# spacejam/tla-rust

Measured on AMD Instinct MI355X. Metric: distinct states/sec, raft.tla (3 servers), higher is better.
Workload: dtype u64

## Files before the change

### __graft_entry__.py

```python
import subprocess
import sys
from pathlib import Path

ROOT = Path(__file__).resolve().parent
sys.path.insert(0, str(ROOT))
sys.path.insert(0, str(ROOT / "tests"))


def build() -> None:
    import tla_rust_amd.build as b
    so = b.build()
    assert so.exists()
    subprocess.run(["make", "-s", "-C", str(ROOT / "oracle")], check=True)
    import helpers
    helpers.build_shim()
    helpers.build_fakerccl()
    helpers.build_tlaeval_door()
    import sgraph
    sgraph.build()
    import sfgraph
    sfgraph.build()
    import ufgraph
    ufgraph.build()
    import sideshim
    sideshim.build()
    sideshim.build_host()
    import behshim
    behshim.build()
    behshim.build_devices()
    import tla_rust_amd
    tla_rust_amd.lib()


def smoke() -> None:
    import helpers
    import tla_rust_amd as amd
    assert amd.device_count() >= 1, "smoke() needs a HIP device"
    for spec, params in (("atomic_add", [10]), ("pcal_intro", [0, 1, 20, 2]), ("raft", [2, 2, 2, 9, 1, 1]), ("ssi", [2, 2, 127, 0])):
        eng = amd.Engine(spec, params, device=0, table_capacity=1 << 20, arena_capacity=1 << 18, chunk_states=1 << 14)
        r = eng.run()
        o = helpers.oracle_run(spec, params)
        assert (r.distinct, r.generated, r.depth, r.verdict, r.levels) == \
               (o["distinct"], o["generated"], o["depth"], o["verdict"], o["levels"]), (spec, dict(r), o)
        eng.close()
        print(f"smoke {spec}{params}: {r.distinct} distinct / {r.generated} generated / depth {r.depth} == oracle")
    params = [0, 3, 2, 3, 15, 3, 1]
    eng = amd.Engine("paxos", params, device=0, table_capacity=1 << 20, arena_capacity=1 << 18, deadlock=False)
    r = eng.run()
    o = helpers.oracle_run("paxos", params, check_deadlock=False)
    assert (r.distinct, r.generated, r.depth, r.verdict, r.levels) == (o["distinct"], o["generated"], o["depth"], o["verdict"], o["levels"])
    assert r.distinct == 17153
    eng.close()
    print(f"smoke paxos{params}: {r.distinct} orbits / {r.generated} generated / depth {r.depth} == oracle == reference text")
    sys.path.insert(0, str(ROOT / "oracle"))
    from tla_eval import Checker
    text = (ROOT / "specs" / "pluscal" / "cas_counter.tla").read_text()
    prog = amd.Program(text, (ROOT / "specs" / "pluscal" / "cas_counter.cfg").read_text())
    eng = amd.Engine("pcal", prog.params, device=0, table_capacity=1 << 20, arena_capacity=1 << 18, chunk_states=1 << 12)
    r = eng.run()
    o = Checker(prog.translated(), constants={"Workers": 2, "N": 2}).run_levels(invariants=["NeverTooMany", "SeenIsOld"])
    assert (r.distinct, r.generated, r.depth, r.verdict, r.levels) == (o["distinct"], o["generated"], o["depth"], o["verdict"], o["levels"])
    eng.close()
# ... 9 lines not shown
```

### include/tlamc.h

```cpp
#ifndef TLAMC_H
#define TLAMC_H
#include <stddef.h>
#include <stdint.h>

#ifdef __cplusplus
extern "C" {
#endif

#define MC_OK 0
#define MC_EBADCFG (-1)
#define MC_EHIP (-2)
#define MC_EOVERFLOW (-3)
#define MC_ETABLEFULL (-4)
#define MC_EARENA (-5)
#define MC_ERCCL (-6)
#define MC_ESTATE (-7)
#define MC_EPARSE (-8)
#define MC_ENOSPEC (-9)
#define MC_EROUTE (-10)

#define MC_V_OK 0
#define MC_V_INVARIANT 1
#define MC_V_ASSERT 2
#define MC_V_DEADLOCK 3
#define MC_V_SPECERR 4
#define MC_V_BUDGET 5
#define MC_V_ASSUME 6
#define MC_V_LIVENESS 7

#define MC_SPEC_ATOMIC_ADD 1
#define MC_SPEC_PCAL_INTRO 2
#define MC_SPEC_RAFT 3

#define MC_SPEC_SSI 4

#define MC_SPEC_PCAL 5

#define MC_SPEC_PAXOS 6

typedef struct {
    uint32_t spec_id;
    uint32_t nparams;
    int64_t params[16];
} mc_spec_desc;

#define MC_F_DEADLOCK 1u
#define MC_F_TRACE 2u
#define MC_F_TIMING 4u
#define MC_F_MATRIX 8u
#define MC_F_NOPROBE 16u
#define MC_F_NOFAMILY 32u
#define MC_F_OCC3 2048u
#define MC_F_NOINWAVE 65536u
#define MC_F_WAVETAIL 131072u
#define MC_F_PARK 32768u
#define MC_F_NOFILTER 8192u
#define MC_F_SYNCPROBE 4096u
#define MC_F_PROGRESS 16384u
#define MC_F_NOBATCH 256u
#define MC_F_UNVERIFIED 512u
#define MC_F_JIT 262144u
#define MC_F_GENERIC 128u
#define MC_F_STRONGFAIR 33554432u
#define MC_F_LABELFAIR 134217728u
#define MC_F_COVERAGE 16777216u
#define MC_F_CONTINUE 67108864u

typedef struct {
    int32_t device;
    uint32_t flags;
    uint64_t table_capacity;
    uint64_t arena_capacity;
    uint64_t chunk_states;
    uint64_t max_levels;
    uint64_t max_distinct;
    uint32_t shard_rank;
    uint32_t shard_count;
} mc_config;

#define MC_MAX_LEVELS 4096

typedef struct {
    uint64_t distinct;
    uint64_t generated;
    uint64_t queue_left;
    uint32_t depth;
    int32_t verdict;
    int32_t violated_invariant;
    uint32_t trace_len;
    uint32_t levels;
// ... 371 lines not shown
```

### tla_rust_amd/build.py

```python
import os
import subprocess
from pathlib import Path

PKG = Path(__file__).resolve().parent
CSRC = PKG / "csrc"
OUT = PKG / "_build"
LIB = OUT / "libtlamc.so"
CLI = OUT / "mc"

SOURCES = ["engine.hip", "frontend.cpp"]

ENGINE_BASE = ["engine.hip", "hip_owned.h", "engine_kernels.h", "engine_sim.h", "sim_walk.h", "engine_behaviours.h", "behaviour.h", "engine_coverage.h", "coverage.h", "engine_violations.h", "violations.h",
               "engine_graph.h",
               "graph.h", "liveness.h", "live_query.h", "state_graph.h", "spec_gen.h", "mc_common.h", "spec_registry.h", "../../include/tlamc.h"]
ENGINE_OWN = {0: ["spec_pluscal.h", "spec_raft.h", "spec_raft_packed.h", "spec_ssi.h", "spec_vm.h", "spec_vm_cfg.h", "spec_paxos.h", "engine_pairs.h"], 7: ["spec_paxos.h"], 1: ["spec_pluscal.h"],
              2: ["spec_raft.h"], 3: ["spec_raft.h"], 4: ["spec_raft.h"], 5: ["spec_ssi.h", "engine_pairs.h"], 6: ["spec_vm.h", "spec_vm_cfg.h"],
              12: ["spec_raft.h", "spec_raft_packed.h"], 13: ["spec_raft.h", "spec_raft_packed.h"]}
STATE_GRAPH_DEPS = ["state_graph.hip", "state_graph.h", "engine_live.h", "hip_owned.h", "liveness.h", "live_query.h", "graph.h", "coverage.h", "mc_common.h", "spec_registry.h",
                    "spec_gen.h", "spec_pluscal.h", "spec_raft.h", "spec_raft_packed.h", "spec_ssi.h", "spec_vm.h", "spec_vm_cfg.h", "spec_paxos.h", "../../include/tlamc.h"]


def _stale(target, deps):
    if not target.exists():
        return True
    t = target.stat().st_mtime
    return any(d.stat().st_mtime > t for d in deps)


def build(force=False, verbose=False):
    OUT.mkdir(exist_ok=True)
    hipcc = os.environ.get("HIPCC", "/opt/rocm/bin/hipcc")
    deps = list(CSRC.glob("*")) + [PKG.parent / "include" / "tlamc.h"]
    srcs = [str(CSRC / s) for s in SOURCES if (CSRC / s).exists()]
    common = [hipcc, "--offload-arch=gfx950", "-O3", "-std=c++17", "-fPIC", "-Wno-unused-value", "-Wno-unused-result",
              "-I", str(PKG.parent / "include")]
    if os.environ.get("TLAMC_LINE_TABLES"):
        common.append("-gline-tables-only")
    if os.environ.get("TLAMC_EXTRA_DEFS"):
        common += os.environ["TLAMC_EXTRA_DEFS"].split()
    if os.environ.get("TLAMC_PHASE_PROF"):
        common.append("-DMC_PHASE_PROF")
    jobs, objs = [], []
    for tu in sorted(ENGINE_OWN):
        obj = OUT / f"engine_tu{tu}.o"
        objs.append(obj)
# ... 48 lines not shown
```

### tla_rust_amd/csrc/engine.hip

```cpp
#include <hip/hip_runtime.h>

#include <algorithm>
#include <chrono>
#include <memory>
#include <type_traits>
#include <string>
#include <vector>

#include "spec_registry.h"
#include "hip_owned.h"

namespace mc {

#ifndef MC_TU
#define MC_TU -1
#endif
}
#include "engine_kernels.h"
#include "engine_pairs.h"
#include "engine_sim.h"
#include "engine_behaviours.h"
#include "engine_coverage.h"
#include "engine_violations.h"
#include "engine_graph.h"
#include "state_graph.h"
namespace mc {

struct EngineBase {
    DevBuf<int32_t> owned_device_blob;
    uint64_t program_hash = 0;
    mc_progress_fn progress_fn = nullptr;
    void *progress_user = nullptr;
    double progress_interval = 1.0;
    std::chrono::steady_clock::time_point progress_last;
    bool stop_requested = false;
    void report_progress(uint32_t levels, uint64_t generated, uint64_t distinct, uint64_t queue) {
        if (!progress_fn) return;
        const auto now = std::chrono::steady_clock::now();
        if (std::chrono::duration<double>(now - progress_last).count() < progress_interval) return;
        progress_last = now;
        progress_fn(progress_user, levels, generated, distinct, queue);
    }
    virtual ~EngineBase() = default;
    virtual int run(mc_result *out) = 0;
    virtual int step(uint32_t levels, mc_result *out) = 0;
    virtual int trace(uint8_t *states_out, int32_t *actions_out, size_t *n_inout) = 0;
    virtual int kernel_stats(mc_kernel_stats *out) = 0;
    virtual int read_states(uint64_t first, uint64_t count, uint8_t *out) = 0;
    virtual int debug_reexpand(unsigned extra_flags, double *ms) = 0;
    virtual int debug_phases(uint64_t *out48, int reset) = 0;
    virtual int debug_flags(uint32_t set, uint32_t clear) = 0;
// ... 710 lines not shown
        const unsigned gm = bx < 8 * 256 ? (bx + 7) / 8 : 256;
        return gm ? gm : 1u;
    }
    void finish_materialise(uint64_t chunk_base, uint64_t ncols, unsigned parity, hipStream_t expanded_on = nullptr) {
        if (pairs_only()) return;
        unsigned gm = mat_grid(ncols);
        if (fr.mat_inwave_level) {
            const uint64_t want = (fr.mat_list_hint * 4 + 255) / 256;
            const unsigned per_seg = (unsigned)((want + NSHARD - 1) / NSHARD);
            if (per_seg < gm) gm = per_seg ? per_seg : 1u;
        }
        hipEventRecord(ev_e[parity].get(), expanded_on ? expanded_on : stream.s);
        hipStreamWaitEvent(stream2, ev_e[parity].get(), 0);
        timed(2, 0, [&] {
            hipLaunchKernelGGL(k_materialise<S>, dim3(gm, NSHARD), dim3(256), 0, stream2, prm, d_arena, chunk_base, d_newlist,
                               seg_cap, arena_cap, d_parent, d_pslot, d_ctr, parity, (const LevelCtl *)nullptr, (const uint64_t *)d_newfp);
        }, stream2);
        hipLaunchKernelGGL(k_commit, dim3(1), dim3(1), 0, stream2, d_ctr, parity);
        hipEventRecord(ev_m[parity].get(), stream2);
        static const bool serial = getenv("TLAMC_SERIAL") != nullptr;
        if (serial) hipStreamSynchronize(stream2);
    }
    void enqueue_blind_level(uint64_t max_states) {
        const uint64_t ncols = max_states + 64;
        RouteArgs rt{};
        rt.lc = d_lc;
        rt.new_fp = d_newfp;
        set_inwave(rt);
        const unsigned sg = slices_for(ncols, true);
        const bool dl = sg > 1 && (cfg.flags & MC_F_DEADLOCK);
        if (dl) { rt.succ = d_nsl; hipMemsetAsync(d_nsl, 0, ncols * sizeof(uint16_t), stream); }
        const unsigned lflags = cfg.flags | ((cfg.flags & MC_F_PARK) ? MC_FI_PARK : 0u);
        timed(0, 0, [&] {
            launch_expand<S, false>(!(cfg.flags & MC_F_NOFAMILY), lflags, ncols, stream, sg, prm, (const uint64_t *)d_arena,
                                    (uint64_t)0, (uint64_t)0, ncols, d_table.p, seen_arg(), d_newlist.p, seg_cap, d_ctr.p, cfg.flags, rt, 0u);
            if (dl) hipLaunchKernelGGL(k_deadlock_slices, dim3((unsigned)((ncols + 255) / 256)), dim3(256), 0, stream, (const uint16_t *)d_nsl,
                                       (uint64_t)0, (uint64_t)0, ncols, (const LevelCtl *)d_lc, d_ctr);
        });
        if (!pairs_only()) timed(2, 0, [&] {
            hipLaunchKernelGGL(k_materialise<S>, dim3(32, NSHARD), dim3(256), 0, stream, prm, d_arena, (uint64_t)0, d_newlist, seg_cap,
                               arena_cap, d_parent, d_pslot, d_ctr, 0u, (const LevelCtl *)d_lc, (const uint64_t *)d_newfp);
        });
        hipLaunchKernelGGL(k_end_level, dim3(1), dim3(1), 0, stream, d_ctr, d_lc);
    }

    template <bool INIT>
    void finish_chunk(uint64_t chunk_base_or_first, uint64_t ncols, unsigned rows) {
        const unsigned bx = (unsigned)((ncols + 255) / 256);
        timed(1, ncols * rows, [&] {
            hipLaunchKernelGGL(k_insert, dim3(bx, rows), dim3(256), 0, stream, d_cand, row_stride, ncols, d_nsl, d_table,
                               seen_arg(), d_newlist, d_ctr);
        });
        const unsigned gm = bx < 2048 ? bx : 2048;
        timed(2, 0, [&] {
            if (INIT)
                hipLaunchKernelGGL(k_init_materialise<S>, dim3(gm), dim3(256), 0, stream, prm, d_arena, chunk_base_or_first,
                                   d_inittmp, d_newlist, arena_cap, d_parent, d_pslot, d_ctr);
            else
                hipLaunchKernelGGL(k_materialise<S>, dim3(gm, 1), dim3(256), 0, stream, prm, d_arena, chunk_base_or_first,
                                   d_newlist, seg_cap, arena_cap, d_parent, d_pslot, d_ctr, 0u, (const LevelCtl *)nullptr, (const uint64_t *)nullptr);
        });
        hipLaunchKernelGGL(k_commit, dim3(1), dim3(1), 0, stream, d_ctr, 0u);
    }

    int seed_init(unsigned rank, unsigned count, bool resuming, bool in_place, std::chrono::steady_clock::time_point *t0) {
        if (!in_place) HIP_TRY(hipMemsetAsync(d_table, 0, table_cap * sizeof(uint64_t), stream));
        HIP_TRY(hipMemsetAsync(d_ctr, 0, sizeof(DevCounters), stream));
// ... 126 lines not shown
                alloc_atomic = lvl_inwave;
            }
            prev_frontier = hi - lo;
            fr.mat_inwave_level = lvl_inwave;
            unsigned chunk_no = 0;
            const bool two_streams = stream_b && !use_matrix && hi - lo > chunk && !(slices_for(chunk, false) > 1 && (cfg.flags & MC_F_DEADLOCK));
            if (two_streams) {
                hipEventRecord(ev_level.get(), stream);
                hipStreamWaitEvent(stream_b, ev_level.get(), 0);
            }
            for (uint64_t c0 = lo; c0 < hi; ++chunk_no) {
                const unsigned parity = chunk_no & 1u;
                const uint64_t base = c0 & ~63ull;
                uint64_t c1 = base + chunk;
                if (c1 > hi) c1 = hi;
                const uint64_t ncols = ((c1 - base) + 63) & ~63ull;
                if (use_matrix) {
                    timed(0, c1 - c0, [&] {
                        hipLaunchKernelGGL(k_expand<S>, dim3((unsigned)((ncols + 255) / 256)), dim3(256), 0, stream, prm, d_arena,
                                           c0, c1, d_cand, row_stride, ncols, d_nsl, d_ctr, cfg.flags);
                    });
                    finish_chunk<false>(base, ncols, max_slots);
                } else {
                    hipStream_t es = two_streams && parity ? stream_b.s : stream.s;
                    if (chunk_no >= 2) hipStreamWaitEvent(es, ev_m[parity].get(), 0);
                    RouteArgs rt_new{};
                    rt_new.new_fp = d_newfp;
                    if (lvl_inwave) set_inwave(rt_new);
                    const unsigned sg = slices_for(ncols, false);
                    const bool dl = sg > 1 && (cfg.flags & MC_F_DEADLOCK);
                    if (dl) { rt_new.succ = d_nsl; hipMemsetAsync(d_nsl, 0, ncols * sizeof(uint16_t), es); }
                    const unsigned lflags = cfg.flags | (lvl_inwave && park_levels ? MC_FI_PARK : 0u);
                    timed(0, c1 - c0, [&] {
                        launch_expand<S, false>(!(cfg.flags & MC_F_NOFAMILY), lflags, ncols, es, sg, prm,
                                                (const uint64_t *)d_arena, c0, c1, ncols, d_table.p, seen_arg(), d_newlist.p, seg_cap, d_ctr.p,
                                                cfg.flags, rt_new, parity);
                        if (dl) hipLaunchKernelGGL(k_deadlock_slices, dim3((unsigned)((ncols + 255) / 256)), dim3(256), 0, es,
                                                   (const uint16_t *)d_nsl, c0, c1, ncols, (const LevelCtl *)nullptr, d_ctr);
                    }, es);
                    finish_materialise(base, ncols, parity, es);
                }
                c0 = c1;
            }
            if ((rc = read_counters())) return rc;
            if ((rc = check_dev_error())) return rc;
            {
                const uint64_t via = h_ctr->via_list - via_seen;
                via_seen = h_ctr->via_list;
                const double growth = hi > lo ? (double)(h_ctr->arena_next - hi) / (double)(hi - lo) : 1.0;
                fr.mat_list_hint = (uint64_t)((double)(via / (chunk_no ? chunk_no : 1u)) * (growth > 1.0 ? growth : 1.0)) + 1;
            }
            if (cov.on) { cov_generated(lo, hi); cov_distinct(hi, h_ctr->arena_next); }
            if (vio.on && h_ctr->viol_key != ~0ull && (rc = viol_level(lo, hi, h_ctr->arena_next, true))) return rc;
            if ((rc = close_level(lo, hi, h_ctr->arena_next, level, out))) return rc;
            progress(level, lo, hi);
        }
        if (cov.on && (rc = cov_end())) return rc;
        if (hi > lo && h_ctr->viol_key == ~0ull && !fr.stop_frontier && (rc = check_frontier(lo, hi))) return rc;
        if (vio.on && hi > lo && !vio.fatal && h_ctr->viol_key != ~0ull && (rc = viol_level(lo, hi, hi, false))) return rc;
        const unsigned long long run_key = vio.on && vio.have_first ? vio.first_key : h_ctr->viol_key;
        const auto t1 = std::chrono::steady_clock::now();
        out->seconds = std::chrono::duration<double>(t1 - t0).count();
        out->distinct = h_ctr->arena_next;
        fr.last_distinct = h_ctr->arena_next;
        kstat[2].units = h_ctr->arena_next;
        out->generated = 0;
        fr.cells = 0;
// ... 296 lines not shown
                e1 = hipMemcpyAsync(out + off * W * sizeof(uint64_t), tmp, n * W * sizeof(uint64_t), hipMemcpyDeviceToHost, stream);
                e2 = hipStreamSynchronize(stream);
            }
            if (e1 != hipSuccess || e2 != hipSuccess) { set_error("read_states: copy failed"); return MC_EHIP; }
        }
        return MC_OK;
    }
    int debug_flags(uint32_t set, uint32_t clear) override { cfg.flags = (cfg.flags & ~clear) | set; return MC_OK; }
    int seen_layout(uint64_t *buckets, uint32_t *slots) override {
        *buckets = seen_arg() & ~SEEN_SPARSE;
        *slots = seen_sparse ? MC_SPARSE_SLOTS : 8;
        return MC_OK;
    }
    int debug_phases(uint64_t *out48, int reset) override {
#ifdef MC_PHASE_PROF
        HIP_TRY(hipSetDevice(cfg.device));
        HIP_TRY(hipDeviceSynchronize());
        HIP_TRY(hipMemcpyFromSymbol(out48, HIP_SYMBOL(g_phase), 48 * sizeof(uint64_t)));
        if (reset) { static const unsigned long long zero[48] = {}; HIP_TRY(hipMemcpyToSymbol(HIP_SYMBOL(g_phase), zero, sizeof zero)); }
        return MC_OK;
#else
        (void)out48; (void)reset;
        set_error("the library was built without MC_PHASE_PROF");
        return MC_ESTATE;
#endif
    }
    int debug_reexpand(unsigned extra_flags, double *ms) override {
        HIP_TRY(hipSetDevice(cfg.device));
        Event a(hipEventDefault), b(hipEventDefault);
        HIP_TRY(hipEventRecord(a.get(), stream));
        for (uint64_t c0 = 0; c0 < fr.last_distinct; c0 += chunk) {
            const uint64_t c1 = c0 + chunk < fr.last_distinct ? c0 + chunk : fr.last_distinct;
            const uint64_t ncols = ((c1 - c0) + 63) & ~63ull;
            launch_expand<S, false>(!((cfg.flags | extra_flags) & MC_F_NOFAMILY), cfg.flags | extra_flags, ncols, stream, 0u, prm,
                                    (const uint64_t *)d_arena, c0, c1, ncols, d_table.p, seen_arg(), d_newlist.p, seg_cap, d_ctr.p,
                                    cfg.flags | extra_flags, RouteArgs{}, 0u);
            hipLaunchKernelGGL(k_commit, dim3(1), dim3(1), 0, stream, d_ctr, 0u);
        }
        HIP_TRY(hipEventRecord(b.get(), stream));
        HIP_TRY(hipStreamSynchronize(stream));
        float t = 0;
        HIP_TRY(hipEventElapsedTime(&t, a.get(), b.get()));
        *ms = t;
        return MC_OK;
    }
    int shard_alloc(ShSlot &q, uint64_t send_cap) {
        const unsigned P = nranks();
        if (send_cap > q.pend_src.n) {
            q.rt_fp.reset(); q.rt_src.reset(); q.pend_src.reset();
            q.rt_subcap = (send_cap / (P * NSHARD)) * 2 + 4096;
            HIP_TRY(q.rt_fp.alloc((size_t)P * NSHARD * q.rt_subcap));
            HIP_TRY(q.rt_src.alloc((size_t)P * NSHARD * q.rt_subcap));
            HIP_TRY(q.pend_src.alloc(send_cap));
        }
        HIP_TRY(q.rt_cur.reserve((size_t)(P * NSHARD)));
        if (send_cap > sh.d_incl.n) {
            sh.d_new_src.reset(); sh.d_incl.reset();
            HIP_TRY(sh.d_new_src.alloc(send_cap));
            HIP_TRY(sh.d_incl.alloc(send_cap));
        }
        HIP_TRY(sh.d_ends.reserve(8));
        HIP_TRY(sh.h_ends.reserve(8));
        HIP_TRY(sh.h_cur.reserve((size_t)8 * NSHARD));
        return MC_OK;
    }
    static int refuse_packed() {
        if constexpr (PackedRows<S>::value) { set_error("this engine of generated code stores rows packed to its program's cell ranges and serves ONE GPU: create a sharded engine with shard_count > 1 (or $TLAMC_JIT_PACK=0)"); return MC_EBADCFG; }
// ... 106 lines not shown
            hipLaunchKernelGGL(k_materialise<S>, dim3(mat_grid(q.ncols), NSHARD), dim3(256), 0, stream2, prm, d_arena, q.chunk_base, d_newlist, seg_cap,
                               arena_cap, d_parent, d_pslot, d_ctr, slot, (const LevelCtl *)nullptr, (const uint64_t *)d_newfp);
        }, stream2);
        hipLaunchKernelGGL(k_commit, dim3(1), dim3(1), 0, stream2, d_ctr, slot);
        append_end(stream2);
        HIP_TRY(hipEventRecord(sh.ev_mat[slot].get(), stream2));
        return MC_OK;
    }
    int shard_expand_launch(unsigned slot, uint64_t first, uint64_t count, uint64_t send_cap) override {
        HIP_TRY(hipSetDevice(cfg.device));
        if (slot > 1) { set_error("shard_expand: slot must be 0 or 1"); return MC_EBADCFG; }
        ShSlot &q = sh.sl[slot];
        const unsigned P = nranks();
        int rc = shard_alloc(q, send_cap);
        if (rc) return rc;
        q.pend_total = 0;
        q.count = count;
        q.launched = true;
        for (unsigned t = 0; t <= 8; t++) q.pend_off.off[t] = 0;
        if (first + count > sh.hi - sh.lo) { set_error("shard_expand: chunk outside the local frontier"); return MC_EBADCFG; }
        if (count > chunk) { set_error("shard_expand: chunk larger than chunk_states"); return MC_EBADCFG; }
        if (!count) return MC_OK;
        if (sh.ev_slot[slot].made()) HIP_TRY(hipStreamWaitEvent(stream, sh.ev_slot[slot].get(), 0));
        if (sh.ev_mat[slot].made()) HIP_TRY(hipStreamWaitEvent(stream, sh.ev_mat[slot].get(), 0));
        HIP_TRY(hipMemsetAsync(q.rt_cur, 0, (size_t)(P * NSHARD) * sizeof(PaddedCounter), stream));
        const uint64_t c0 = sh.lo + first, c1 = c0 + count, base = c0 & ~63ull;
        const uint64_t ncols = ((c1 - base) + 63) & ~63ull;
        q.chunk_base = base;
        RouteArgs rt{P, q.rt_cur, q.rt_fp, q.rt_src, q.rt_subcap};
        rt.my_rank = cfg.shard_rank;
        rt.new_fp = d_newfp;
        q.ncols = ncols;
        timed(0, count, [&] {
            launch_expand<S, true>(!(cfg.flags & MC_F_NOFAMILY), cfg.flags, ncols, stream, 0u, prm,
                                   (const uint64_t *)d_arena, c0, c1, ncols, d_table.p, seen_arg(), d_newlist.p, seg_cap, d_ctr.p, cfg.flags, rt, slot);
        });
        return MC_OK;
    }
    int shard_expand_finish(unsigned slot, uint64_t *send_fp, uint64_t send_cap, uint64_t *send_counts) override {
        HIP_TRY(hipSetDevice(cfg.device));
        if (slot > 1 || !sh.sl[slot].launched) { set_error("shard_expand_finish: no expand in flight for this slot"); return MC_EBADCFG; }
        ShSlot &q = sh.sl[slot];
        q.launched = false;
        const unsigned P = nranks();
        for (unsigned t = 0; t < P; t++) send_counts[t] = 0;
        if (!q.count) return MC_OK;
        PaddedCounter *cur = sh.h_cur;
        HIP_TRY(hipMemcpyAsync(cur, q.rt_cur, (size_t)(P * NSHARD) * sizeof(PaddedCounter), hipMemcpyDeviceToHost, stream));
        HIP_TRY(hipMemcpyAsync(h_ctr, d_ctr, sizeof(DevCounters), hipMemcpyDeviceToHost, stream));
        HIP_TRY(hipStreamSynchronize(stream));
        int rc;
        if ((rc = check_dev_error())) return rc;
        uint64_t total = 0;
        for (unsigned t = 0; t < P; t++) {
            q.pend_off.off[t] = total;
            for (unsigned x = 0; x < NSHARD; x++) {
                if (cur[t * NSHARD + x].v > q.rt_subcap) { set_error("shard_expand: route bucket overflow (raise send_cap)"); return MC_EROUTE; }
                send_counts[t] += cur[t * NSHARD + x].v;
            }
            total += send_counts[t];
        }
        for (unsigned t = P; t <= 8; t++) q.pend_off.off[t] = total;
        if (total >= (1ull << 31)) { set_error("shard_expand: more than 2^31 candidates in one round (lower chunk_states)"); return MC_EARENA; }
        if (total > q.pend_src.n) { set_error("shard_expand: more candidates in one round than the slot's pending list holds (raise the fan-out allowance)"); return MC_EROUTE; }
        if (total > send_cap) { set_error("shard_expand: send buffer too small (raise the fan-out allowance)"); return MC_EROUTE; }
        q.pend_total = total;
        if (q.keep_pending) {
// ... 1025 lines not shown
```

Baseline: 4.234 billion.

## Add specialized production expand kernel for small Raft specs with cold kernarg reloads

Adds a dedicated family-expand kernel for Raft specs with at most three servers, used when no generic or debug flags are set. Rarely used arguments are re-read from the kernarg segment only where needed, to cut register pressure and spills. The kernel also uses a batched seen-set insert: one vectorized first-round bucket probe per lane, with a non-inlined narrow fallback that only runs when the first round cannot place the fingerprint. This duplicates a large kernel body, which raises maintenance cost and the risk of diverging from the generic path. A register and spill inspection script and a new flag that forces the generic path are added as well.

```diff
diff --git a/__graft_entry__.py b/__graft_entry__.py
--- a/__graft_entry__.py
+++ b/__graft_entry__.py
@@ -28,6 +28,9 @@
     import behshim
     behshim.build()
     behshim.build_devices()
+    import probeshim
+    probeshim.build()
+    probeshim.build_host()
     import tla_rust_amd
     tla_rust_amd.lib()
 
diff --git a/include/tlamc.h b/include/tlamc.h
--- a/include/tlamc.h
+++ b/include/tlamc.h
@@ -56,6 +56,7 @@
 #define MC_F_PARK 32768u
 #define MC_F_NOFILTER 8192u
 #define MC_F_SYNCPROBE 4096u
+#define MC_F_GENERICEXPAND 268435456u
 #define MC_F_PROGRESS 16384u
 #define MC_F_NOBATCH 256u
 #define MC_F_UNVERIFIED 512u
diff --git a/profiles/kspill.py b/profiles/kspill.py
--- /dev/null
+++ b/profiles/kspill.py
@@ -0,0 +1,137 @@
+#!/usr/bin/env python
+import json
+import re
+import subprocess
+import sys
+import tempfile
+from pathlib import Path
+
+LLVM = "/opt/rocm/lib/llvm/bin/"
+META = ("vgpr_count", "sgpr_count", "vgpr_spill_count", "sgpr_spill_count", "group_segment_fixed_size", "private_segment_fixed_size")
+
+
+def _demangle(names):
+    out = subprocess.run(["c++filt"], input="\n".join(names), capture_output=True, text=True).stdout.splitlines()
+    return dict(zip(names, out))
+
+
+def _disasm_counts(co, wanted):
+    txt = subprocess.run([LLVM + "llvm-objdump", "-d", "--no-show-raw-insn", str(co)], capture_output=True, text=True).stdout
+    per = {}
+    cur = None
+    for ln in txt.splitlines():
+        m = re.match(r"^[0-9a-f]+ <(.+)>:$", ln)
+        if m:
+            cur = m.group(1) if m.group(1) in wanted else None
+            if cur:
+                per[cur] = []
+            continue
+        if cur is None:
+            continue
+        ins = ln.split("//")[0].strip()
+        if ins:
+            per[cur].append(ins)
+    res = {}
+    for name, lines in per.items():
+        stores, spill_regs = 0, set()
+        for ins in lines:
+            m = re.match(r"v_writelane_b32\s+(v\d+)", ins)
+            if m:
+                stores += 1
+                spill_regs.add(m.group(1))
+        reloads = 0
+        for ins in lines:
+            m = re.match(r"v_readlane_b32\s+\S+\s+(v\d+)", ins)
+            if m and m.group(1) in spill_regs:
+                reloads += 1
+        res[name] = {"lane_reloads": reloads, "lane_stores": stores, "scalar_spill_vgprs": sorted(spill_regs, key=lambda r: int(r[1:])),
+                     "s_nop": sum(1 for i in lines if i.startswith("s_nop")),
+                     "valu_insts": sum(1 for i in lines if i.startswith("v_")),
+                     "salu_insts": sum(1 for i in lines if i.startswith("s_") and not i.startswith(("s_nop", "s_waitcnt", "s_load", "s_buffer_load"))),
+                     "cmpswap_sites": sum(1 for i in lines if "atomic_cmpswap" in i),
+                     "insts": len(lines)}
+    return res
+
+
+def _code_objects(obj, d):
+    fat = Path(d) / "f.bin"
+    subprocess.run([LLVM + "llvm-objcopy", "--dump-section", f".hip_fatbin={fat}", str(obj), str(Path(d) / "copy.o")], check=True)
+    blob, magic = fat.read_bytes(), b"__CLANG_OFFLOAD_BUNDLE__"
+    starts = [m.start() for m in re.finditer(re.escape(magic), blob)]
+    out = []
+    for n, a in enumerate(starts):
+        piece, co = Path(d) / f"b{n}.bin", Path(d) / f"k{n}.co"
+        piece.write_bytes(blob[a:starts[n + 1] if n + 1 < len(starts) else len(blob)])
+        r = subprocess.run([LLVM + "clang-offload-bundler", "--unbundle", "--type=o", f"--input={piece}", "--targets=hipv4-amdgcn-amd-amdhsa--gfx950", f"--output={co}"],
+                           capture_output=True)
+        if r.returncode == 0 and co.exists() and co.stat().st_size:
+            out.append(co)
+    return out
+
+
+def _records(co):
+    notes = subprocess.run([LLVM + "llvm-readelf", "--notes", str(co)], capture_output=True, text=True).stdout
+    recs, cur, args = [], {}, []
+    for ln in notes.splitlines():
+        m = re.match(r"\s+(?:- )?\.(\w+):\s+(.*)", ln)
+        if not m:
+            continue
+        k, v = m.groups()
+        if k == "offset":
+            args.append([int(v), None, None])
+        elif k == "size" and args:
+            args[-1][1] = int(v)
+        elif k == "value_kind" and args:
+            args[-1][2] = v
+        elif k == "name" and v.startswith("_Z"):
+            cur["symbol"] = v
+        elif k in META:
+            cur[k] = int(v)
+        if k == "wavefront_size":
+            if "symbol" in cur:
+                cur["args"] = [tuple(a) for a in args if a[2] and not a[2].startswith("hidden")]
+                recs.append(cur)
+            cur, args = {}, []
+    return recs
+
+
+def kernels(obj, flt="expand_family", disasm=True):
+    out = []
+    with tempfile.TemporaryDirectory() as d:
+        for co in _code_objects(obj, d):
+            recs = _records(co)
+            if not recs:
+                continue
+            dem = _demangle([r["symbol"] for r in recs])
+            recs = [r for r in recs if flt in dem[r["symbol"]]]
+            if not recs:
+                continue
+            size = {}
+            for ln in subprocess.run([LLVM + "llvm-readelf", "-sW", str(co)], capture_output=True, text=True).stdout.splitlines():
+                f = ln.split()
+                if len(f) >= 8 and f[3] == "FUNC":
+                    size[f[7]] = int(f[2])
+            counts = _disasm_counts(co, {r["symbol"] for r in recs}) if disasm else {}
+            for r in recs:
+                k = {"kernel": re.sub(r"\(.*", "", dem[r["symbol"]]).replace("void ", ""), "sgpr_count": r.get("sgpr_count"), "sgpr_spill_count": r.get("sgpr_spill_count"),
+                     "vgpr_count": r.get("vgpr_count"), "vgpr_spill_count": r.get("vgpr_spill_count"), "scratch_bytes": r.get("private_segment_fixed_size"),
+                     "lds_bytes": r.get("group_segment_fixed_size"), "code_bytes": size.get(r["symbol"]), "args": r["args"]}
+                k.update(counts.get(r["symbol"], {}))
+                out.append(k)
+    return out
+
+
+def main():
+    args = [a for a in sys.argv[1:] if a != "--json"]
+    ks = kernels(args[0], args[1] if len(args) > 1 else "expand_family")
+    if "--json" in sys.argv:
+        print(json.dumps([{a: b for a, b in k.items() if a != "args"} for k in ks], indent=1))
+        return
+    for k in ks:
+        print(f"{k['kernel']}\n    sgpr {k['sgpr_count']} (spill {k['sgpr_spill_count']})  vgpr {k['vgpr_count']} (spill {k['vgpr_spill_count']})  scratch {k['scratch_bytes']}  "
+              f"LDS {k['lds_bytes']}  code {k['code_bytes']} B\n    lane reloads {k.get('lane_reloads')}  lane stores {k.get('lane_stores')}  on {k.get('scalar_spill_vgprs')}  "
+              f"s_nop {k.get('s_nop')}  v_* {k.get('valu_insts')}  s_* {k.get('salu_insts')}  cmpswap {k.get('cmpswap_sites')}  insts {k.get('insts')}")
+
+
+if __name__ == "__main__":
+    main()
diff --git a/tla_rust_amd/build.py b/tla_rust_amd/build.py
--- a/tla_rust_amd/build.py
+++ b/tla_rust_amd/build.py
@@ -10,7 +10,7 @@
 
 SOURCES = ["engine.hip", "frontend.cpp"]
 
-ENGINE_BASE = ["engine.hip", "hip_owned.h", "engine_kernels.h", "engine_sim.h", "sim_walk.h", "engine_behaviours.h", "behaviour.h", "engine_coverage.h", "coverage.h", "engine_violations.h", "violations.h",
+ENGINE_BASE = ["engine.hip", "hip_owned.h", "engine_kernels.h", "engine_expand_prod.h", "seen_batch.h", "engine_sim.h", "sim_walk.h", "engine_behaviours.h", "behaviour.h", "engine_coverage.h", "coverage.h", "engine_violations.h", "violations.h",
                "engine_graph.h",
                "graph.h", "liveness.h", "live_query.h", "state_graph.h", "spec_gen.h", "mc_common.h", "spec_registry.h", "../../include/tlamc.h"]
 ENGINE_OWN = {0: ["spec_pluscal.h", "spec_raft.h", "spec_raft_packed.h", "spec_ssi.h", "spec_vm.h", "spec_vm_cfg.h", "spec_paxos.h", "engine_pairs.h"], 7: ["spec_paxos.h"], 1: ["spec_pluscal.h"],
diff --git a/tla_rust_amd/csrc/engine.hip b/tla_rust_amd/csrc/engine.hip
--- a/tla_rust_amd/csrc/engine.hip
+++ b/tla_rust_amd/csrc/engine.hip
@@ -17,6 +17,7 @@
 #endif
 }
 #include "engine_kernels.h"
+#include "engine_expand_prod.h"
 #include "engine_pairs.h"
 #include "engine_sim.h"
 #include "engine_behaviours.h"
@@ -793,7 +794,7 @@
         if (dl) { rt.succ = d_nsl; hipMemsetAsync(d_nsl, 0, ncols * sizeof(uint16_t), stream); }
         const unsigned lflags = cfg.flags | ((cfg.flags & MC_F_PARK) ? MC_FI_PARK : 0u);
         timed(0, 0, [&] {
-            launch_expand<S, false>(!(cfg.flags & MC_F_NOFAMILY), lflags, ncols, stream, sg, prm, (const uint64_t *)d_arena,
+            launch_expand_default<S, false>(!(cfg.flags & MC_F_NOFAMILY), lflags, ncols, stream, sg, prm, (const uint64_t *)d_arena,
                                     (uint64_t)0, (uint64_t)0, ncols, d_table.p, seen_arg(), d_newlist.p, seg_cap, d_ctr.p, cfg.flags, rt, 0u);
             if (dl) hipLaunchKernelGGL(k_deadlock_slices, dim3((unsigned)((ncols + 255) / 256)), dim3(256), 0, stream, (const uint16_t *)d_nsl,
                                        (uint64_t)0, (uint64_t)0, ncols, (const LevelCtl *)d_lc, d_ctr);
@@ -986,7 +987,7 @@
                     if (dl) { rt_new.succ = d_nsl; hipMemsetAsync(d_nsl, 0, ncols * sizeof(uint16_t), es); }
                     const unsigned lflags = cfg.flags | (lvl_inwave && park_levels ? MC_FI_PARK : 0u);
                     timed(0, c1 - c0, [&] {
-                        launch_expand<S, false>(!(cfg.flags & MC_F_NOFAMILY), lflags, ncols, es, sg, prm,
+                        launch_expand_default<S, false>(!(cfg.flags & MC_F_NOFAMILY), lflags, ncols, es, sg, prm,
                                                 (const uint64_t *)d_arena, c0, c1, ncols, d_table.p, seen_arg(), d_newlist.p, seg_cap, d_ctr.p,
                                                 cfg.flags, rt_new, parity);
                         if (dl) hipLaunchKernelGGL(k_deadlock_slices, dim3((unsigned)((ncols + 255) / 256)), dim3(256), 0, es,
@@ -1349,7 +1350,7 @@
         for (uint64_t c0 = 0; c0 < fr.last_distinct; c0 += chunk) {
             const uint64_t c1 = c0 + chunk < fr.last_distinct ? c0 + chunk : fr.last_distinct;
             const uint64_t ncols = ((c1 - c0) + 63) & ~63ull;
-            launch_expand<S, false>(!((cfg.flags | extra_flags) & MC_F_NOFAMILY), cfg.flags | extra_flags, ncols, stream, 0u, prm,
+            launch_expand_default<S, false>(!((cfg.flags | extra_flags) & MC_F_NOFAMILY), cfg.flags | extra_flags, ncols, stream, 0u, prm,
                                     (const uint64_t *)d_arena, c0, c1, ncols, d_table.p, seen_arg(), d_newlist.p, seg_cap, d_ctr.p,
                                     cfg.flags | extra_flags, RouteArgs{}, 0u);
             hipLaunchKernelGGL(k_commit, dim3(1), dim3(1), 0, stream, d_ctr, 0u);
@@ -1522,7 +1523,7 @@
         rt.new_fp = d_newfp;
         q.ncols = ncols;
         timed(0, count, [&] {
-            launch_expand<S, true>(!(cfg.flags & MC_F_NOFAMILY), cfg.flags, ncols, stream, 0u, prm,
+            launch_expand_default<S, true>(!(cfg.flags & MC_F_NOFAMILY), cfg.flags, ncols, stream, 0u, prm,
                                    (const uint64_t *)d_arena, c0, c1, ncols, d_table.p, seen_arg(), d_newlist.p, seg_cap, d_ctr.p, cfg.flags, rt, slot);
         });
         return MC_OK;
diff --git a/tla_rust_amd/csrc/engine_expand_prod.h b/tla_rust_amd/csrc/engine_expand_prod.h
--- /dev/null
+++ b/tla_rust_amd/csrc/engine_expand_prod.h
@@ -0,0 +1,390 @@
+#ifndef TLAMC_ENGINE_EXPAND_PROD_H
+#define TLAMC_ENGINE_EXPAND_PROD_H
+
+namespace mc {
+
+#include "seen_batch.h"
+static_assert(SEEN_BATCH_SPARSE == SEEN_SPARSE && SEEN_BATCH_ETABLE == DEV_ETABLE, "seen_batch.h and engine_kernels.h disagree about the mode bit or the error bit");
+
+constexpr unsigned EXPAND_GENERIC_BITS = MC_F_NOPROBE | 64u  | MC_F_NOFILTER | MC_F_SYNCPROBE | MC_F_WAVETAIL | MC_F_GENERICEXPAND | MC_F_OCC3 | MC_FI_PARK;
+template <class S>
+struct ExpandProd : std::false_type {};
+template <int NS>
+struct ExpandProd<SpecRaft<NS>> : std::integral_constant<bool, (NS <= 3)> {};
+template <int NS>
+struct ExpandProd<SpecRaftPacked<NS>> : std::integral_constant<bool, (NS <= 3)> {};
+
+template <class P>
+struct ExpandKernargs {
+    P prm;
+    const uint64_t *arena;
+    uint64_t lo, hi, ncols;
+    uint64_t *table;
+    uint64_t mask;
+    uint32_t *newlist;
+    uint64_t seg_cap;
+    DevCounters *ctr;
+    unsigned flags;
+    RouteArgs rt;
+    unsigned parity;
+};
+struct ExpandCold {
+    const uint64_t *arena;
+    uint64_t lo, hi, ncols;
+    uint32_t *newlist;
+    uint64_t seg_cap;
+    DevCounters *ctr;
+    unsigned flags;
+    uint64_t *new_fp, *arena_w;
+    uint64_t arena_cap;
+    uint32_t *parent;
+    uint16_t *pslot;
+    unsigned parity;
+};
+template <class P>
+__device__ __forceinline__ ExpandCold expand_cold_args() {
+    typedef const __attribute__((address_space(4))) ExpandKernargs<P> *KP;
+    uint64_t a = (uint64_t)__builtin_amdgcn_kernarg_segment_ptr();
+    asm volatile("" : "+s"(a));
+    const KP k = (KP)a;
+    ExpandCold c{k->arena, k->lo, k->hi, k->ncols, k->newlist, k->seg_cap, k->ctr, k->flags & ~EXPAND_GENERIC_BITS, k->rt.new_fp, k->rt.arena_w, k->rt.arena_cap,
+                 k->rt.parent, k->rt.pslot, k->parity};
+    const LevelCtl *lc = k->rt.lc;
+    if (lc) {
+        c.lo = lc->lo;
+        c.hi = lc->hi;
+        c.ncols = ((c.hi - (c.lo & ~63ull)) + 63) & ~63ull;
+    }
+    return c;
+}
+template <class S, int MINW = MC_EXPAND_MINW, int WAVES = MC_EXPAND_WAVES>
+__global__ void __launch_bounds__(64 * WAVES, MINW)
+k_expand_family_prod(typename S::Params prm, const uint64_t *__restrict__ arena, uint64_t lo, uint64_t hi, uint64_t ncols,
+                     uint64_t *table, uint64_t mask, uint32_t *__restrict__ newlist, uint64_t seg_cap, DevCounters *ctr, unsigned flags,
+                     RouteArgs rt, unsigned parity) {
+    constexpr int NB = 1;
+    static_assert(WAVES == 1 || WAVES == 2 || WAVES == 4, "wavefronts per workgroup");
+    using FamLdsT = FamLds<S, NB>;
+    __shared__ FamQueues wq[WAVES];
+    __shared__ FamLdsT fls[WAVES];
+    (void)newlist; (void)seg_cap; (void)ctr; (void)parity;
+    if (rt.lc) {
+        if (rt.lc->stop) return;
+        lo = rt.lc->lo;
+        hi = rt.lc->hi;
+        ncols = ((hi - (lo & ~63ull)) + 63) & ~63ull;
+    }
+    const unsigned lane = threadIdx.x & 63;
+    FamQueues &Q = wq[threadIdx.x >> 6];
+    FamLdsT &FL = fls[threadIdx.x >> 6];
+    const uint64_t base = lo & ~63ull;
+    const uint64_t wave_col0 = ((uint64_t)blockIdx.x * WAVES + (threadIdx.x >> 6)) * (64ull * NB);
+    const bool inwave = rt.arena_w != nullptr;
+    if (wave_col0 >= ncols && !inwave) return;
+    const uint64_t wave_idx0 = base + wave_col0;
+    const int W = S::words(prm);
+    static_assert(NB == 1, "BlockRef addresses ONE arena block per wavefront");
+    const GlobalWords blk_base = uniform_ptr(arena + (wave_idx0 >> 6) * (uint64_t)W * 64);
+    unsigned long long viol = ~0ull;
+    unsigned gen = 0, err = 0, cands = 0;
+    unsigned qhead = 0, qn = 0, ohead = 0, on = 0;
+#pragma unroll
+    for (int t = 0; t < WFILT / 64; ++t) FL.filt[t * 64 + lane] = 0;
+    bool track_succ = (flags & MC_F_DEADLOCK) != 0;
+    bool lane_succ = false;
+    uint64_t fheadA = 0, fheadB = 0, fcntA = 0, fcntB = 0;
+    auto fget = [](uint64_t a, uint64_t b, int f) -> unsigned { return (unsigned)((f < 8 ? a >> (8 * f) : b >> (8 * (f - 8))) & 255u); };
+    auto fset = [](uint64_t &a, uint64_t &b, int f, unsigned v) {
+        if (f < 8) a = (a & ~(255ull << (8 * f))) | ((uint64_t)v << (8 * f));
+        else b = (b & ~(255ull << (8 * (f - 8)))) | ((uint64_t)v << (8 * (f - 8)));
+    };
+    const unsigned okeep = inwave ? (unsigned)(OCAP - 64) : 63u;
+    __shared__ unsigned wg_park[WAVES];
+    __shared__ unsigned wg_hist_s[WAVES * SlotClasses<S>::value];
+    __shared__ unsigned long long wg_out0_s;
+
+    auto flush_out = [&](unsigned take) __attribute__((always_inline)) {
+        const unsigned e = lane < take ? Q.o_ent[owrap(ohead + lane)] : O_DEAD;
+        const unsigned long long bl = __ballot(e != O_DEAD);
+        unsigned long long pos = 0;
+        const ExpandCold C = expand_cold_args<typename S::Params>();
+        const unsigned pshard = C.parity * NSHARD + (blockIdx.x & (NSHARD - 1));
+        uint32_t *__restrict__ seg = C.newlist + (uint64_t)pshard * C.seg_cap;
+        const uint64_t col0 = ((uint64_t)blockIdx.x * WAVES + (threadIdx.x >> 6)) * (64ull * NB);
+        if (lane == 0 && bl) pos = atomicAdd(&C.ctr->n_new[pshard].v, (unsigned long long)__popcll(bl));
+        pos = __shfl(pos, 0) + (unsigned)__popcll(bl & ((1ull << lane) - 1ull));
+        if (e != O_DEAD) {
+            seg[pos] = (uint32_t)(col0 + (e & 63u)) | ((uint32_t)(e >> 6) << 24);
+            if (C.new_fp) C.new_fp[(uint64_t)pshard * C.seg_cap + pos] = Q.o_fp[owrap(ohead + lane)];
+        }
+        ohead = owrap(ohead + take);
+        on -= take;
+    };
+    auto flush_probe = [&](unsigned take) __attribute__((always_inline)) {
+        unsigned src = 0;
+        uint64_t qfp = 0;
+        if (lane < take) {
+            const unsigned k = (qhead + lane) & (QCAP - 1);
+            src = Q.q_ent[k];
+            qfp = Q.q_fp[k];
+        }
+        const bool is_new = seen_insert_batch(table, mask, qfp, lane < take, err);
+        qhead = (qhead + take) & (QCAP - 1);
+        qn -= take;
+        const unsigned long long b = __ballot(is_new);
+        if (is_new) {
+            const unsigned k = owrap(ohead + on + (unsigned)__popcll(b & ((1ull << lane) - 1ull)));
+            Q.o_ent[k] = (uint16_t)src;
+            Q.o_fp[k] = qfp;
+        }
+        on += (unsigned)__popcll(b);
+        wave_lds_fence();
+        if (on > okeep) flush_out(64);
+    };
+    auto fam_push = [&](int f, unsigned long long b, bool mine, unsigned entry) __attribute__((always_inline)) -> bool {
+        const unsigned h = fget(fheadA, fheadB, f), c = fget(fcntA, fcntB, f);
+        if (mine) FL.fq[f][(h + c + (unsigned)__popcll(b & ((1ull << lane) - 1ull))) & (FQCAP - 1)] = (uint16_t)entry;
+        const unsigned nc = c + (unsigned)__popcll(b);
+        fset(fcntA, fcntB, f, nc);
+        return nc >= 64;
+    };
+    auto enqueue = [&](uint64_t fp, unsigned src , int back_to) __attribute__((always_inline)) {
+        const unsigned long long b0 = __ballot(fp != 0);
+        if (b0) {
+            cands += (unsigned)__popcll(b0);
+            if (fp) {
+                const unsigned h = (unsigned)(fp >> 20) & (WFILT - 1);
+                if (FL.filt[h] == fp) fp = 0;
+                else FL.filt[h] = fp;
+            }
+            const unsigned long long b = __ballot(fp != 0);
+            const unsigned nb = (unsigned)__popcll(b);
+            if (fp) {
+                const unsigned k = (qhead + qn + (unsigned)__popcll(b & ((1ull << lane) - 1ull))) & (QCAP - 1);
+                Q.q_fp[k] = fp;
+                Q.q_ent[k] = (uint16_t)src;
+            }
+            qn += nb;
+            wave_lds_fence();
+            if (qn >= 64) flush_probe(64);
+        }
+        (void)back_to;
+    };
+    auto run_family = [&](int f, unsigned take, int back_to) __attribute__((always_inline)) {
+        const unsigned h = fget(fheadA, fheadB, f);
+        wave_lds_fence();
+        uint64_t fp = 0;
+        unsigned src = 0;
+        if (lane < take) {
+            const unsigned e = FL.fq[f][(h + lane) & (FQCAP - 1)];
+            const unsigned p = e & 255u;
+            const int slot = (int)(e >> 8);
+            const uint64_t pidx = wave_idx0 + p;
+            const typename S::Summary q = FL.sum[p];
+            const BlockRef sp{blk_base, p & 63u};
+            unsigned st = 0;
+            uint64_t fv = 0;
+            family_dispatch<S, 0>(f, [&](auto fc) { st = S::template eval_pair<decltype(fc)::value>(prm, q, sp, slot, fv); });
+            if (st & ST_ENABLED) {
+                ++gen;
+                if (track_succ) atomicOr(S::succ_word(FL.sum[p]), 0x80000000u);
+                if (st & ST_OVERFLOW) err |= DEV_EOVERFLOW;
+                else if (st & ST_ASSERT) viol = min(viol, viol_key(pidx, (unsigned)slot, VK_ASSERT, 0));
+                else if (st & ST_SPECERR) viol = min(viol, viol_key(pidx, (unsigned)slot, VK_SPECERR, 0));
+                else {
+                    if (st & ST_INVARIANT) viol = min(viol, viol_key(pidx, (unsigned)slot, VK_INVARIANT, st >> 8));
+                    if (!(st & (ST_OUT_OF_MODEL | ST_SELFLOOP))) { fp = fv; src = ((unsigned)slot << 6) | (p & 63u); }
+                }
+            }
+        }
+        fset(fheadA, fheadB, f, (h + take) & (FQCAP - 1));
+        fset(fcntA, fcntB, f, fget(fcntA, fcntB, f) - take);
+        enqueue(fp, src, back_to);
+        wave_lds_fence();
+    };
+    auto run_full = [&](unsigned fullmask, bool drain, int back_to) __attribute__((always_inline)) {
+        while (fullmask) {
+            const int f = __ffs((int)fullmask) - 1;
+            const unsigned c = fget(fcntA, fcntB, f);
+            run_family(f, drain ? (c < 64 ? c : 64u) : 64u, back_to);
+            if (fget(fcntA, fcntB, f) < (drain ? 1u : 64u)) fullmask &= ~(1u << f);
+        }
+    };
+
+    for (int blk = 0; blk < NB; ++blk) {
+        const uint64_t idx = wave_idx0 + (uint64_t)blk * 64 + lane;
+        if (wave_col0 + (uint64_t)blk * 64 >= ncols) break;
+        const bool active = idx >= lo && idx < hi;
+        const unsigned pl = (unsigned)blk * 64 + lane;
+        const BlockRef g{blk_base, lane};
+        typename S::Guards gd;
+        gd.fixed = gd.fixed_hi = 0;
+        gd.infl = 0;
+        int nm = 0;
+        typename S::Local loc;
+        if (active) {
+            S::load_expand(prm, g, loc, gd);
+            nm = loc.nm;
+            typename S::Summary q;
+            S::summarize(loc, q);
+            FL.sum[pl] = q;
+            const unsigned ps = S::parent_status(prm, loc, g);
+            if (ps & ST_INVARIANT) viol = min(viol, viol_key(idx, SLOT_PARENT, VK_INVARIANT, ps >> 8));
+        }
+        wave_lds_fence();
+        const int wnm = (int)wave_max_u32((unsigned)nm);
+        if constexpr (DenseSlots<S>::value > 0) {
+            {
+                bool mysucc = false;
+#pragma clang loop unroll(disable)
+                for (int i = 0; i < S::DENSE_PAIRS; ++i) {
+                    unsigned st2[2] = {0u, 0u};
+                    uint64_t f2[2] = {0ull, 0ull};
+                    if (active) S::eval_dense(prm, loc, g, i, st2[0], f2[0], st2[1], f2[1]);
+#pragma unroll
+                    for (int h = 0; h < 2; ++h) {
+                        const unsigned st = st2[h];
+                        const unsigned slot = (unsigned)S::dense_slot(i, h);
+                        uint64_t fp = 0;
+                        if (st & ST_ENABLED) {
+                            ++gen;
+                            mysucc = true;
+                            if (st & ST_OVERFLOW) err |= DEV_EOVERFLOW;
+                            else if (st & ST_ASSERT) viol = min(viol, viol_key(idx, slot, VK_ASSERT, 0));
+                            else if (st & ST_SPECERR) viol = min(viol, viol_key(idx, slot, VK_SPECERR, 0));
+                            else {
+                                if (st & ST_INVARIANT) viol = min(viol, viol_key(idx, slot, VK_INVARIANT, st >> 8));
+                                if (!(st & (ST_OUT_OF_MODEL | ST_SELFLOOP))) fp = f2[h];
+                            }
+                        }
+                        enqueue(fp, (slot << 6) | pl, 1);
+                    }
+                }
+                S::fixed_clear_dense(gd);
+                if (track_succ) {
+                    lane_succ = mysucc;
+                    if (!__ballot(active && !mysucc)) track_succ = false;
+                }
+            }
+        }
+        static_assert(InlineMsgs<S>::value, "a by-family spec evaluates its message actions inline (S::inflight_slots)");
+        {
+            {
+                unsigned infl = active ? S::inflight_slots(gd) : 0u;
+                auto eval_three = [&](bool on, int k) __attribute__((always_inline)) {
+#pragma clang loop unroll(disable)
+                    for (int kind = 0; kind < 3; ++kind) {
+                        const unsigned slot = (unsigned)(S::FIX + 3 * k + kind);
+                        uint64_t fv = 0, fp = 0;
+                        bool ev = on;
+                        if constexpr (HasGeneratedOnly<S>::value) {
+                            if (on && S::message_generated_only(prm, loc, g, (int)slot)) {
+                                ++gen;
+                                lane_succ = true;
+                                ev = false;
+                            }
+                        }
+                        const unsigned st = ev ? S::eval(prm, loc, g, (int)slot, fv) : 0u;
+                        if (st & ST_ENABLED) {
+                            ++gen;
+                            lane_succ = true;
+                            if (st & ST_OVERFLOW) err |= DEV_EOVERFLOW;
+                            else if (st & ST_ASSERT) viol = min(viol, viol_key(idx, slot, VK_ASSERT, 0));
+                            else if (st & ST_SPECERR) viol = min(viol, viol_key(idx, slot, VK_SPECERR, 0));
+                            else {
+                                if (st & ST_INVARIANT) viol = min(viol, viol_key(idx, slot, VK_INVARIANT, st >> 8));
+                                if (!(st & (ST_OUT_OF_MODEL | ST_SELFLOOP))) fp = fv;
+                            }
+                        }
+                        enqueue(fp, (slot << 6) | pl, 6);
+                    }
+                };
+                while (__ballot(infl != 0)) {
+                    const bool on = infl != 0;
+                    const int k = on ? __ffs((int)infl) - 1 : 0;
+                    infl &= infl - 1;
+                    eval_three(on, k);
+                }
+                for (int k = S::GUARD_SLOTS; k < wnm; ++k) {
+                    const bool on = k < nm && S::m_count(S::rd_msg(g, k)) > 0;
+                    if (__ballot(on)) eval_three(on, k);
+                }
+            }
+        }
+        const int lane_inflight = active ? loc.inflight : 0;
+        for (int step = 0; step < S::FIX; ++step) {
+            const int f = S::fixed_family(step);
+            bool en = S::fixed_bit(gd, step);
+            if constexpr (HasGeneratedOnly<S>::value) {
+                if (en && S::fixed_generated_only(prm, lane_inflight, step)) {
+                    ++gen;
+                    lane_succ = true;
+                    en = false;
+                }
+            }
+            const unsigned long long b = __ballot(en);
+            if (b && fam_push(f, b, en, ((unsigned)step << 8) | pl)) run_full(1u << f, false, 5);
+        }
+    }
+    {
+        unsigned fullmask = 0;
+#pragma unroll
+        for (int f = 0; f < S::NFAM; ++f) if (fget(fcntA, fcntB, f)) fullmask |= 1u << f;
+        run_full(fullmask, true, 7);
+    }
+    if (qn) flush_probe(qn);
+    if (inwave) {
+        constexpr int NCLS = SlotClasses<S>::value;
+        static_assert(NCLS * WAVES <= 64, "one lane per (class, wavefront) in the prefix sum");
+        static_assert(sizeof(fls[0].fq) % 8 == 0 && offsetof(FamLdsT, filt) == sizeof(fls[0].fq), "the filter lies directly behind the family queues");
+        static_assert(WAVES * OCAP * sizeof(uint16_t) <= sizeof(fls[0].fq) + sizeof(fls[0].filt), "the sorted order aliases the family queues + the duplicate filter of the first wavefront");
+        uint16_t *order = reinterpret_cast<uint16_t *>(&fls[0].fq[0][0]);
+        const ExpandCold C = expand_cold_args<typename S::Params>();
+        const uint64_t wg_idx0 = (C.lo & ~63ull) + (uint64_t)blockIdx.x * (64u * WAVES);
+        tail_round<S, WAVES, false>(prm, C.arena, C.arena_w, C.arena_cap, C.parent, C.pslot, C.ctr, C.flags, &wq[0], &fls[0], &wg_hist_s[0], (unsigned)NCLS, &wg_out0_s,
+                                    order, &wg_park[0], threadIdx.x >> 6, lane, wg_idx0, ohead, on, err, [](int) {});
+    } else if (on) {
+        flush_out(on);
+    }
+
+    const ExpandCold CE = expand_cold_args<typename S::Params>();
+    if (CE.flags & MC_F_DEADLOCK) {
+        wave_lds_fence();
+        const uint64_t col0 = ((uint64_t)blockIdx.x * WAVES + (threadIdx.x >> 6)) * (64ull * NB);
+        const uint64_t idx = (CE.lo & ~63ull) + col0 + lane;
+        if (col0 < CE.ncols && idx >= CE.lo && idx < CE.hi && !lane_succ && !(*S::succ_word(FL.sum[lane]) >> 31)) viol = min(viol, viol_key(idx, SLOT_NONE, VK_DEADLOCK, 0));
+    }
+    const unsigned gsum = wave_sum_u32(gen);
+    const unsigned long long vmin = wave_min_u64(viol);
+    const unsigned eor = wave_or_u32(err);
+    if (lane == 0) {
+        const unsigned shard = blockIdx.x & (NSHARD - 1);
+        if (gsum) atomicAdd(&CE.ctr->generated[shard].v, (unsigned long long)gsum);
+        if (cands) atomicAdd(&CE.ctr->cells[shard].v, (unsigned long long)cands);
+        if (vmin != ~0ull) atomicMin(&CE.ctr->viol_key, vmin);
+        if (eor) atomicOr(&CE.ctr->error, eor);
+    }
+}
+
+template <class P>
+using ExpandKernelFn = void (*)(decltype(ExpandKernargs<P>::prm), decltype(ExpandKernargs<P>::arena), decltype(ExpandKernargs<P>::lo), decltype(ExpandKernargs<P>::hi),
+                                decltype(ExpandKernargs<P>::ncols), decltype(ExpandKernargs<P>::table), decltype(ExpandKernargs<P>::mask), decltype(ExpandKernargs<P>::newlist),
+                                decltype(ExpandKernargs<P>::seg_cap), decltype(ExpandKernargs<P>::ctr), decltype(ExpandKernargs<P>::flags), decltype(ExpandKernargs<P>::rt),
+                                decltype(ExpandKernargs<P>::parity));
+template <class S, bool ROUTE, class... A>
+static void launch_expand_default(bool by_family, unsigned flags, uint64_t ncols, hipStream_t stream, unsigned slices, A... args) {
+    if constexpr (!ROUTE && ExpandProd<S>::value) {
+        if (by_family && !(flags & EXPAND_GENERIC_BITS)) {
+            constexpr unsigned WG = 64u * MC_EXPAND_WAVES;
+            static_assert(std::is_same<decltype(&k_expand_family_prod<S>), ExpandKernelFn<typename S::Params>>::value,
+                          "k_expand_family_prod's arguments are ExpandKernargs' members, in their order");
+            hipLaunchKernelGGL((k_expand_family_prod<S>), dim3((unsigned)((ncols + WG - 1) / WG)), dim3(WG), 0, stream, args...);
+            return;
+        }
+    }
+    launch_expand<S, ROUTE>(by_family, flags, ncols, stream, slices, args...);
+}
+
+}
+
+#endif
diff --git a/tla_rust_amd/csrc/seen_batch.h b/tla_rust_amd/csrc/seen_batch.h
--- /dev/null
+++ b/tla_rust_amd/csrc/seen_batch.h
@@ -0,0 +1,94 @@
+#ifndef TLAMC_SEEN_BATCH_H
+#define TLAMC_SEEN_BATCH_H
+
+#ifndef MC_NT_PROBE
+#define MC_NT_PROBE 0
+#endif
+#ifndef MC_SEEN_ROTATE
+#define MC_SEEN_ROTATE 1
+#endif
+#ifndef MC_SPARSE_SLOTS
+#define MC_SPARSE_SLOTS 4
+#endif
+constexpr uint64_t SEEN_BATCH_SPARSE = 1ull << 63;
+constexpr unsigned SEEN_BATCH_ETABLE = 1u;
+#if MC_NT_PROBE & 1
+typedef unsigned long long mc_batch_ull2 __attribute__((ext_vector_type(2)));
+#endif
+
+template <int SLOTS>
+__device__ __forceinline__ unsigned seen_first_round(uint64_t *table, uint64_t nbuckets, uint64_t fp) {
+    const uint64_t b = (((fp & 0xffffffffull) * nbuckets) >> 32) * SLOTS;
+    unsigned long long slot[SLOTS];
+#if MC_NT_PROBE & 1
+    const mc_batch_ull2 *line = reinterpret_cast<const mc_batch_ull2 *>(table + b);
+#pragma unroll
+    for (int i = 0; i < SLOTS / 2; ++i) { const mc_batch_ull2 v = __builtin_nontemporal_load(line + i); slot[2 * i] = v.x; slot[2 * i + 1] = v.y; }
+#else
+    const ulonglong2 *line = reinterpret_cast<const ulonglong2 *>(table + b);
+#pragma unroll
+    for (int i = 0; i < SLOTS / 2; ++i) { const ulonglong2 v = line[i]; slot[2 * i] = v.x; slot[2 * i + 1] = v.y; }
+#endif
+    unsigned zm = 0;
+    bool hit = false;
+#pragma unroll
+    for (int i = 0; i < SLOTS; ++i) {
+        hit |= slot[i] == fp;
+        zm |= (slot[i] == 0 ? 1u : 0u) << i;
+    }
+#if MC_SEEN_ROTATE
+    const unsigned j0 = (unsigned)(fp >> 32) & (unsigned)(SLOTS - 1);
+    const unsigned rot = ((zm >> j0) | (zm << (SLOTS - j0))) & ((1u << SLOTS) - 1u);
+#else
+    const unsigned j0 = 0, rot = zm;
+#endif
+    unsigned r = hit ? 0u : 2u;
+    if (!hit && rot) {
+        const unsigned i = ((unsigned)__builtin_ctz(rot) + j0) & (unsigned)(SLOTS - 1);
+        const unsigned long long cur = atomicCAS((unsigned long long *)&table[b + i], 0ull, (unsigned long long)fp);
+        r = cur == 0 ? 1u : cur == fp ? 0u : 2u;
+    }
+    return r;
+}
+__device__ __noinline__ unsigned seen_insert_narrow(uint64_t *table, uint64_t nbuckets, uint64_t fp) {
+    const unsigned slots = (nbuckets & SEEN_BATCH_SPARSE) ? (unsigned)MC_SPARSE_SLOTS : 8u;
+    const uint64_t nb = nbuckets & ~SEEN_BATCH_SPARSE;
+    uint64_t bk = ((fp & 0xffffffffull) * nb) >> 32;
+#if MC_SEEN_ROTATE
+    const unsigned j0 = (unsigned)(fp >> 32) & (slots - 1u);
+#else
+    const unsigned j0 = 0;
+#endif
+#pragma clang loop unroll(disable)
+    for (int probe = 0; probe < 2048; ++probe) {
+        unsigned long long *const b = (unsigned long long *)table + bk * slots;
+#pragma clang loop unroll(disable)
+        for (unsigned r = 0; r < slots; ++r) {
+            const unsigned i = (j0 + r) & (slots - 1u);
+            unsigned long long cur = b[i];
+            if (cur == 0ull) cur = atomicCAS(&b[i], 0ull, (unsigned long long)fp);
+            if (cur == 0ull) return 1u;
+            if (cur == fp) return 0u;
+        }
+        bk = bk + 1 == nb ? 0 : bk + 1;
+    }
+    return 2u;
+}
+__device__ __forceinline__ bool seen_insert_batch(uint64_t *table, uint64_t nbuckets, uint64_t fp, bool valid, unsigned &err) {
+    unsigned r = 0;
+    if (nbuckets & SEEN_BATCH_SPARSE) {
+        if (valid) r = seen_first_round<MC_SPARSE_SLOTS>(table, nbuckets & ~SEEN_BATCH_SPARSE, fp);
+    } else {
+        if (valid) r = seen_first_round<8>(table, nbuckets, fp);
+    }
+    if (__ballot(r == 2u)) {
+        if (r == 2u) {
+            const unsigned s = seen_insert_narrow(table, nbuckets, fp);
+            if (s & 2u) err |= SEEN_BATCH_ETABLE;
+            r = s & 1u;
+        }
+    }
+    return r == 1u;
+}
+
+#endif
```

Measured after the change: 4.293 billion, median of 6. 1.4% higher.
